# nalcala/MIDASPOM

Hardware: AMD Instinct MI355X
Metric: grid-point x timestep likelihood evals/sec (higher is better)
Workload: dtype f64; 1 GPU; config2: 64 patches x 50 years, 512x512 (e,c) grid; patches=64, years=50, nvar=8, nstates=256, nextid=40, parallelism=e-row slabs x1, layout=[c][e] (MDP_LAYOUT_CE, the drop-ins' layout)

## Files before the change

midaspom_amd/csrc/spom_engine.h:

```cpp
#ifndef MDP_SPOM_ENGINE_H
#define MDP_SPOM_ENGINE_H

#include <hip/hip_runtime_api.h>
#include <hip/hip_vector_types.h>

#include <cstddef>
#include <cstdint>
#include <map>
#include <mutex>
#include <set>
#include <string>
#include <vector>

#include "mdp_internal.h"
#include "spom_jit.h"

constexpr int kBlock = 256;
constexpr int kEPL = 2;
constexpr int kMaxDeg = 24;
constexpr uint32_t kSubPart = 16;
constexpr uint32_t kOffBits = 22;
constexpr uint32_t kOffMask = (1u << kOffBits) - 1u;
constexpr size_t kFwdLds = 48 * 1024;
constexpr int kZTermsDev = 8;
// ... 17 lines not shown
constexpr int kJitKblockTall = 512;

struct LaunchNote {
    const char *fmt;
    uint64_t a[4];
};

struct DevCtx {
    int device = 0;
    mutable std::vector<LaunchNote> noted;
    hipStream_t stream = nullptr;
    double *S = nullptr;
    uint32_t *var_cols = nullptr, *row_col = nullptr;
    uint32_t *pairA = nullptr, *pairB = nullptr, *pairOff = nullptr;
    uint32_t *udesc = nullptr, *prog = nullptr, *pairPart0 = nullptr, *partP = nullptr, *partK0 = nullptr;
    double *e = nullptr, *c = nullptr;
    size_t cap_e = 0, cap_c = 0;
    uint32_t ne = 0, nc = 0;
    uint32_t ne_sform = 0;
    uint32_t *plist = nullptr;
    size_t cap_plist = 0;
    double *elist = nullptr;
    size_t cap_elist = 0;
    uint32_t nlist = 0, nlist_epl = 0;
    bool plist_identity = true;
    double *ZPV = nullptr, *R = nullptr, *out = nullptr, *gpart = nullptr;
    size_t cap_zpv = 0, cap_r = 0, cap_out = 0, cap_gpart = 0;
    unsigned long long *stamps[3] = {nullptr, nullptr, nullptr};
    size_t cap_st[3] = {0, 0, 0};
    size_t nst[3] = {0, 0, 0};
    double *zs = nullptr, *sv = nullptr, *Qrow = nullptr, *Zg = nullptr;
    double *zsq = nullptr;
    double *zc = nullptr;
    size_t cap_zc = 0;
    uint2 *items = nullptr;
    uint2 *qslot = nullptr;
    uint32_t *qlane = nullptr;
    uint32_t *islot = nullptr;
    uint32_t *itemB = nullptr, *qstart = nullptr, *qitem = nullptr;
    size_t cap_zs = 0, cap_zsq = 0, cap_qrow = 0, cap_zg = 0;
    uint32_t zs_len = 0;
    double *coltab = nullptr;
    size_t cap_coltab = 0;
    uint32_t ct_len = 0;
    uint32_t zs_kmax = 0;
    uint32_t qrows_cb = 1;
// ... 152 lines not shown
inline size_t mmt_lds(const mdp_engine *eng)
{
    const MmtShape sh = mmt_shape(eng);
    return ((sh.db ? 2 : 1) * (size_t)sh.rows * mmt_pts(sh.rt) + 2 * ((size_t)eng->maxA + 1) * mmt_ps(sh.rt)) *
           sizeof(double);
}

inline size_t hs_lds(const mdp_engine *eng)
{
    return (((size_t)1 << eng->hs_nb) + eng->hs_nb + 1) * mmt_pts(eng->hs_rt) * sizeof(double);
}

inline size_t qrows_lds(const mdp_engine *eng, uint32_t cb)
{
    const size_t nv = eng->nvar <= 8 ? 8 : eng->nvar <= 16 ? 16 : 24;
    return ((((size_t)cb * eng->nj + 1) & ~(size_t)1) + (size_t)eng->nj * (cb * nv + 2) + (size_t)cb * eng->npl_slots) *
               sizeof(double) +
           ((size_t)eng->ncoef_d + 1 + eng->qitem.size()) * sizeof(uint32_t);
}

inline size_t fused_lds(const mdp_engine *eng, size_t ct_len)
{
    const size_t fc = (size_t)eng->jit_plan.fused_cols;
    return (ct_len + 2 + fc * (eng->nj + eng->nitems + 2 * eng->ldQ)) * sizeof(double);
}

inline size_t wide_lds(const mdp_engine *eng) { return 2 * ((size_t)eng->maxA + 1) * kBlock * sizeof(double); }


int parse_engine_opts(const char *s, EngineOpts &o, bool diag_build);

enum class MdpPlanMode {
    Compile,
    OfflineCheck,
    TablesOnly
};
int mdp_plan_engine(mdp_engine *eng, const mdp_problem *p, size_t lds_max, MdpPlanMode mode, double *jit_t);

void z_split(const mdp_engine *eng, uint32_t js, double cmax, std::vector<double> &large, double *coef,
             std::vector<uint32_t> *cols = nullptr);
std::string jit_source(mdp_engine *eng, int variant);
int jit_build(mdp_engine *eng, int variant);
int jit_build_chunks(mdp_engine *eng);

#endif
```

midaspom_amd/csrc/spom_engine.hip:

```cpp
#include <hip/hip_ext.h>
#include <hip/hip_runtime.h>

#include <algorithm>
#include <chrono>
#include <cmath>
#include <cstdarg>
#include <cstdio>
#include <cstdlib>
#include <cstring>
#include <mutex>
#include <new>
#include <string>
#include <vector>

#include "spom_dev.h"
#include "spom_engine.h"

namespace {

constexpr int kZpvJ = 64;
constexpr int kZpvSlices = 4;
constexpr int kZpvCT = 2;
constexpr int kZpvUnroll = 8;
constexpr int kStampSlots = 8;
// ... 943 lines not shown
        uint32_t g = 0;
        for (uint32_t i = i0; i < i1; i += kQGroup, ++g) {
            double sg = pl[qitem[i]];
            for (uint32_t u = 1; u < kQGroup && i + u < i1; ++u) sg = sg + pl[qitem[i + u]];
#pragma unroll
            for (int l = 0; l < kQLevels; ++l) {
                if ((g >> l) & 1u) {
                    sg = lev[l] + sg;
                } else {
                    lev[l] = sg;
                    break;
                }
            }
        }
        bool have = false;
#pragma unroll
        for (int l = 0; l < kQLevels; ++l)
            if ((g >> l) & 1u) {
                a = have ? lev[l] + a : lev[l];
                have = true;
            }
    }
    Q[(size_t)(c0 + cl) * ldQ + q] = a;
}

typedef double mdp_d4 __attribute__((ext_vector_type(4)));
template <int NPM>
__global__ __launch_bounds__(kMmaThreads) void k_fwd_mma(
    const double *__restrict__ Q, uint32_t ldQ, const uint32_t *__restrict__ np, const uint2 *__restrict__ kt,
    const uint32_t *__restrict__ kbase, const uint32_t *__restrict__ desc, const uint32_t *__restrict__ dbase,
    const uint2 *__restrict__ wplan, uint32_t tmax, double prior0, const double *__restrict__ evals, uint32_t ne,
    uint32_t c0, uint32_t maxA, uint32_t ktmax, uint32_t zslot, double *__restrict__ out, uint32_t ld_out,
    uint32_t out_cs)
{
    constexpr uint32_t PTS = mma_pts(NPM), ROWS = mma_rows(NPM), PS = mma_ps(NPM), RT = PTS / 16;
    static_assert(NPM <= (int)ROWS && NPM <= 256, "state rows");
    extern __shared__ __attribute__((aligned(16))) double mlds[];
    double *Va = mlds, *Vb = mlds + (size_t)ROWS * PTS;
    double *xp = Vb + (size_t)ROWS * PTS, *yp = xp + (size_t)(maxA + 1) * PS;
    const uint32_t lane = threadIdx.x & 63u, wv = __builtin_amdgcn_readfirstlane(threadIdx.x >> 6);
    const uint32_t p0 = blockIdx.x * PTS, ic = c0 + blockIdx.y;
    if (threadIdx.x < PTS) {
        const uint32_t ie = p0 + threadIdx.x;
        const double e = ie < ne ? evals[ie] : 0.0;
        const double x = e > 1.0 ? 1.0 : e, y = 1.0 - x;
        double a = 1.0, b = 1.0;
// ... 1033 lines not shown

int qrows_attrs(const mdp_engine *eng, DevCtx &d)
{
    if (d.qrows_attr_set) return MDP_OK;
    const size_t lds_max = qrows_lds(eng, kQrowsMaxC);
    if (lds_max > 64 * 1024)
        for (const void *fn : {(const void *)k_qrows<8, true, 1>, (const void *)k_qrows<8, false, 1>,
                               (const void *)k_qrows<16, false, 1>, (const void *)k_qrows<24, false, 1>,
                               (const void *)k_qrows<8, true, 2>, (const void *)k_qrows<8, false, 2>,
                               (const void *)k_qrows<16, false, 2>, (const void *)k_qrows<8, true, 4>,
                               (const void *)k_qrows<8, false, 4>})
            HIP_TRY(hipFuncSetAttribute(fn, hipFuncAttributeMaxDynamicSharedMemorySize,
                                        (int)std::min(lds_max, kQrowsLdsMax)));
    d.qrows_attr_set = true;
    return MDP_OK;
}

void free_device(DevCtx &d)
{
    (void)hipSetDevice(d.device);
    void *ptrs[] = {d.S, d.var_cols, d.row_col, d.pairA, d.pairB, d.pairOff, d.udesc, d.prog,
                    d.pairPart0, d.partP, d.partK0, d.e, d.c, d.ZPV, d.R, d.out, d.gpart,
                    d.zs, d.zsq, d.sv, d.Qrow, d.Zg, d.coltab, d.items, d.itemB, d.qstart, d.qitem,
                    d.Pg, d.V, d.np_d, d.udesc_w, d.zc, d.plist, d.elist, d.qslot, d.qlane, d.islot,
                    d.mma_kt, d.mma_kbase, d.mma_desc, d.mma_dbase, d.mma_wplan,
                    d.mmt_kt, d.mmt_ktile, d.mmt_wplan, d.mmt_cidx,
                    d.hs_kt, d.hs_cidx, d.hs_pbase, d.hs_ppos, d.hs_dpos, d.hs_dbase, d.hs_pk,
                    d.hs_wplan, d.hs_pass, d.hs_dpk,
                    d.stamps[0], d.stamps[1], d.stamps[2]};
    for (void *ptr : ptrs)
        if (ptr) (void)hipFree(ptr);
    for (hipEvent_t ev : d.ev) (void)hipEventDestroy(ev);
    for (hipModule_t m : d.jit_mod)
        if (m) (void)hipModuleUnload(m);
    for (hipModule_t m : d.cmod) (void)hipModuleUnload(m);
    for (uint32_t *q : d.cqidx)
        if (q) (void)hipFree(q);
    if (d.vscr) (void)hipFree(d.vscr);
    if (d.stream) (void)hipStreamDestroy(d.stream);
}

std::vector<uint32_t> point_list(const double *e, uint32_t ne, uint32_t epl)
{
    std::vector<uint32_t> s_rows, t_rows;
    for (uint32_t i = 0; i < ne; ++i) {
        const double x = e[i] > 1.0 ? 1.0 : e[i], y = 1.0 - x;
        (x >= y ? t_rows : s_rows).push_back(i);
// ... 102 lines not shown
        uint32_t cb = nc >= 1024 ? 4u : nc >= 512 ? 2u : 1u;
        cb = std::min(cb, eng->nvar <= 8 ? 4u : eng->nvar <= 16 ? 2u : 1u);
        while (cb > 1 && qrows_lds(eng, cb) > kQrowsLdsMax) cb >>= 1;
        d.qrows_cb = cb;
    } else if ((rc = dev_grow(d.ZPV, d.cap_zpv, (size_t)nc * (eng->nvar + 1) * eng->nstates)) ||
               (rc = dev_grow(d.R, d.cap_r, (size_t)nc * ldR_of(eng)))) {
        return rc;
    }
    if (!eng->jit && !eng->wide && !eng->lds_part &&
        (rc = dev_grow(d.gpart, d.cap_gpart, (size_t)nc * eng->partP.size() * (eng->nvar + 1))))
        return rc;
    if (eng->diag) {
        d.nst[0] = eng->jit ? (size_t)nc
                            : (size_t)((eng->nstates + kZpvJ - 1) / kZpvJ) * ((nc + kZpvCT - 1) / kZpvCT);
        d.nst[1] = nc;
        d.nst[2] = (size_t)nc * ((ne + kBlock - 1) / kBlock);
        for (int k = 0; k < 3; ++k) {
            if ((rc = dev_grow(d.stamps[k], d.cap_st[k], d.nst[k] * kStampSlots))) return rc;
            HIP_TRY(hipMemset(d.stamps[k], 0, d.cap_st[k] * sizeof(unsigned long long)));
        }
    }
    if (ne) HIP_TRY(hipMemcpy(d.e, e, ne * sizeof(double), hipMemcpyHostToDevice));
    if (nc) HIP_TRY(hipMemcpy(d.c, c, nc * sizeof(double), hipMemcpyHostToDevice));
    d.ne = ne;
    d.nc = nc;
    return MDP_OK;
}

template <int NP, int DEG, int EPL>
void launch_fwd_epl(const mdp_engine *eng, const DevCtx &d, double *out, OutStrides os, hipStream_t s)
{
    uint32_t se = os.se, sc = os.sc;
    dim3 grid(d.nc, (d.ne + kBlock * EPL - 1) / (kBlock * EPL));
    const uint32_t nprog = (uint32_t)eng->prog.size() - 1;
    note_launch(eng, d, "%s<%d,%d,%d>", eng->fwd_lds ? "k_forward_lds" : "k_forward", NP, DEG, EPL);
    if (eng->fwd_lds)
        MDP_LAUNCH((k_forward_lds<NP, DEG, EPL>), grid, dim3(kBlock), eng->fwd_lds_bytes, s,
                           d.R, ldR_of(eng), d.prog, nprog, eng->np[0], eng->prior0, d.e, d.ne, out, se,
                           sc, d.stamps[2]);
    else
        MDP_LAUNCH((k_forward<NP, DEG, EPL>), grid, dim3(kBlock), 0, s, d.R, ldR_of(eng),
                           d.prog, nprog, eng->np[0], eng->prior0, d.e, d.ne, out, se, sc);
}

template <int NP, int DEG>
void launch_fwd(const mdp_engine *eng, const DevCtx &d, double *out, OutStrides os, hipStream_t s)
// ... 30 lines not shown
        const double *cv = d.c, *ctab = d.coltab;
        uint32_t ctl = d.ct_len, kmax = d.zs_kmax;
        double *vscr = d.vscr;
        uint32_t ldv = d.ldv;
        const uint32_t *qidx = nullptr;
        uint32_t se = os.se, sc = os.sc;
        const uint32_t kb = d.fused ? eng->jit_kblock_fused : d.tall ? (uint32_t)kJitKblockTall : eng->jit_kblock;
        const uint32_t pro = d.fused ? eng->jit_pro_fused : 1u;
        const uint32_t epl = d.fused ? (uint32_t)eng->jit_epl_fused : (uint32_t)eng->jit_epl;
        const uint32_t spl = eng->jit_plan.vlds && (eng->jit_plan.vsplit == 2 || eng->jit_plan.vsplit == 4)
                                 ? (uint32_t)eng->jit_plan.vsplit : 1u;
        const uint32_t *plist = epl > 1 && !d.plist_identity ? d.plist : nullptr;
        uint32_t nlist = epl > 1 ? d.nlist : d.ne;
        if (epl > 1 && ((!plist && !d.plist_identity) || d.nlist_epl % epl))
            return mdp_set_error(MDP_EINVAL, "no point list for %u points per lane", epl);
        const uint64_t gy = (nlist + kb * epl - 1) / (kb * epl);
        const uint32_t fc = d.fused ? (uint32_t)eng->jit_plan.fused_cols : 1u;
        const uint64_t nb = gy * ((d.nc + fc - 1) / fc);
        if (nb * kb * fc * spl > 0xffffffffull)
            return mdp_set_error(MDP_EUNSUPPORTED, "grid %u x %u too large", d.ne, d.nc);
        const double *tab = d.fused ? ctab : Qrow;
        if (plist) ev = d.elist;
        uint32_t nblk = (uint32_t)nb;
        void *args[] = {(void *)&tab,   (void *)&cv,   (void *)&ev,  (void *)&ctl,  (void *)&nlist,
                        (void *)&ne,    (void *)&nc,   (void *)&plist, (void *)&nblk, (void *)&kmax,
                        (void *)&one,   (void *)&qidx, (void *)&out, (void *)&se,   (void *)&sc,
                        (void *)&prior0, (void *)&vscr, (void *)&ldv, (void *)&st};
        if (!eng->chunks.empty()) {
            const size_t nch = d.cfn.size();
            if (nch != eng->chunks.size() || d.cqidx.size() != nch)
                return mdp_set_error(MDP_EHIP, "forward chunks not loaded (%zu of %zu)", nch, eng->chunks.size());
            for (size_t i = 0; i < nch; ++i) {
                qidx = d.cqidx[i];
                HIP_TRY(hipExtModuleLaunchKernel(d.cfn[i], (uint32_t)(nb * kb * spl), 1, 1, kb * spl, 1, 1, 0, s, args,
                                                 nullptr, i == 0 ? t_kev.start : nullptr,
                                                 i + 1 == nch ? t_kev.stop : nullptr, 0));
            }
            note_launch(eng, d, "mdp_fwd_jit<reading,maxA%u,chunks%zu%s>", eng->maxA, nch,
                        eng->chunks[0].qidx.empty() ? "" : ",gather");
            return MDP_OK;
        }
        const uint32_t dyn = d.fused ? (d.ct_len + 2) * (uint32_t)sizeof(double) : 0u;
        HIP_TRY(hipExtModuleLaunchKernel(d.jit_fn[d.fused ? 1 : d.tall ? 2 : 0], (uint32_t)(nb * kb * fc * spl * pro), 1, 1,
                                         kb * fc * spl * pro, 1, 1, dyn, s, args, nullptr, t_kev.start, t_kev.stop, 0));
        note_launch(eng, d, "mdp_fwd_jit<%s,maxA%u>", d.fused ? "fused" : "reading", eng->maxA);
        if (d.tall) note_launch(eng, d, "mdp_fwd_jit<reading,kb%d>", kJitKblockTall);
// ... 634 lines not shown
```

midaspom_amd/csrc/spom_jit.cpp:

```cpp
#include <dlfcn.h>
#include <hip/hip_runtime_api.h>
#include <hip/hiprtc.h>
#include <unistd.h>

#include <cstdio>
#include <cstdlib>
#include <cstring>
#include <map>
#include <set>
#include <atomic>
#include <mutex>
#include <sstream>
#include <algorithm>
#include <cstdint>
#include <string>
#include <sys/stat.h>
#include <type_traits>
#include <vector>

#include "spom_jit.h"

extern "C" hipError_t hipRuntimeGetVersion(int *) __attribute__((weak));

namespace {
// ... 323 lines not shown
         "    double *__restrict__ out, u32 ld_out, u32 out_cs, double prior0,\n"
         "    double *__restrict__ vscr, u32 ldv, unsigned long long *__restrict__ stamps)\n{\n"
      << "    __shared__ __attribute__((aligned(16))) double Ql[2 * FC * LDQ + 2];\n"
      << stamp(6) << stamp(0);
    if (pl.fused) {
        o << "    extern __shared__ __attribute__((aligned(16))) double ct[];\n"
             "    const u32 n2 = ct_len / 2;\n";
        for (uint32_t k = 0; k < nstg; ++k)
            o << "    const u32 si" << k << "_ = threadIdx.x + " << k << " * NT;\n"
              << "    const double2 stg" << k << "_ = ((const double2 *)coltab)[si" << k << "_ < n2 ? si" << k << "_ : 0];\n";
    }
    o <<
         "    const u32 nb = nblk, full = nb & ~7u;\n"
      << (pl.xcd ? "    const u32 lb = blockIdx.x < full ? (blockIdx.x & 7u) * (full >> 3) + (blockIdx.x >> 3) : blockIdx.x;\n"
                 : "    const u32 lb = blockIdx.x + 0 * full;\n") <<
         "    const u32 half = threadIdx.x / KBLOCK, tid = threadIdx.x % KBLOCK;\n"
      << (FC > 1 && SPL == 1 && pl.rot ? "    const u32 tip = (tid + half * (KBLOCK / 2)) % KBLOCK;\n" : "    const u32 tip = tid;\n")
      << (pl.efast ? "    const u32 gy = (nlist + KBLOCK * EPL - 1) / (KBLOCK * EPL), ic0 = lb / gy * FC, by = lb % gy;\n"
                   : "    const u32 ncb = (nc + FC - 1) / FC, ic0 = lb % ncb * FC, by = lb / ncb;\n")
      << (SPL > 1 || FC == 1 ? "    const u32 ic = ic0;\n" : "    const u32 ic = ic0 + half;\n")
      << (SPL > 1 ? "    const double *Qh = Ql;\n" : "    const double *Qh = Ql + half * LDQ;\n");
    const std::string front = std::string(
         "    u32 ie[EPL], pp[EPL];\n    bool st[EPL];\n    double ev[EPL];\n") +
         (EPL == 1 ? "    pp[0] = by * KBLOCK + tip;\n"
                     "    ie[0] = pp[0];\n"
                     "    st[0] = ie[0] < ne;\n"
                     "    ev[0] = evals[st[0] ? ie[0] : 0u];\n"
                   : "    u32 q_[EPL];\n"
                     "#pragma unroll\n"
                     "    for (int i = 0; i < EPL; ++i) {\n"
                     "        pp[i] = by * (KBLOCK * EPL) + tip * EPL + i;\n"
                     "        q_[i] = pp[i] < nlist ? pp[i] : 0x80000000u;\n"
                     "        const u32 j_ = q_[i] & 0x7fffffffu;\n"
                     "        ev[i] = evals[plist ? (pp[i] < nlist ? pp[i] : nlist) : (j_ < ne ? j_ : 0u)];\n"
                     "    }\n"
                     "    if (plist) {\n"
                     "#pragma unroll\n"
                     "        for (int i = 0; i < EPL; ++i) {\n"
                     "            const u32 l_ = plist[pp[i] < nlist ? pp[i] : 0u];\n"
                     "            q_[i] = pp[i] < nlist ? l_ : 0x80000000u;\n"
                     "        }\n"
                     "    }\n"
                     "#pragma unroll\n"
                     "    for (int i = 0; i < EPL; ++i) {\n"
                     "        ie[i] = q_[i] & 0x7fffffffu;\n"
                     "        st[i] = !(q_[i] >> 31) && ie[i] < ne;\n"
                     "    }\n") +
         "#pragma unroll\n"
         "    for (int i = 0; i < EPL; ++i) ev[i] = ie[i] < ne ? ev[i] : 0.0;\n"
         "    asm volatile(\"\" :: \"s\"(kmax), \"s\"(one), \"s\"(out), \"s\"(ld_out), \"s\"(out_cs), \"s\"(prior0), "
         "\"s\"(vscr), \"s\"(ldv));\n";
    std::string wblock;
    {
        std::ostringstream w;
        w << "#pragma unroll\n"
             "    for (int i = 0; i < EPL; ++i) {\n"
             "        const double e = ev[i];\n"
             "        xx[i] = e > 1.0 ? 1.0 : e;\n"
             "        yy[i] = 1.0 - xx[i];\n"
             "    }\n"
             "    const bool tf = xx[0] >= yy[0];\n"
             "    const double *Qp = Qh + (tf ? FC * LDQ : 0);\n"
             "#pragma unroll\n"
             "    for (int i = 0; i < EPL; ++i) {\n"
             "        const double num = tf ? yy[i] : xx[i], den = tf ? xx[i] : yy[i];\n"
             "        zz[i] = num / den;\n"
             "        bb[i] = den;\n"
             "        const double g = tf ? 1.0 : zz[i];\n"
             "        bp[i][0] = 1.0;\n"
             "        gp[i][0] = 1.0;\n"
             "#pragma unroll\n        for (int r = 1; r <= DP; ++r) bp[i][r] = bp[i][r - 1] * den;\n"
             "#pragma unroll\n        for (int r = 1; r <= DG; ++r) gp[i][r] = gp[i][r - 1] * g;\n";
        const char *vdst = pl.vlds ? "Vl[(k * EPL + i) * KBLOCK + tid]" : "v[i][k]";
        const char *kloop = SPL > 1 ? "#pragma unroll\n        for (int k = half; k < NPMAX; k += SPL) "
                                    : "#pragma unroll\n        for (int k = 0; k < NPMAX; ++k) ";
        if (pl.first)
            w << kloop << vdst << " = k < " << np0 << " ? 1.0 : 0.0;\n";
        else
            w << kloop << vdst << " = k < " << np0 << " ? vscr[((size_t)k * nc + ic) * ldv + pp[i]] : 0.0;\n";
        w << "    }\n";
        wblock = w.str();
    }
    const bool w_early = !pl.fused && !pl.first;
    const std::string early_w = w_early ? wblock : std::string();
    o << "    double xx[EPL], yy[EPL], zz[EPL], bb[EPL], bp[EPL][DP + 1], gp[EPL][DG + 1];\n"
         "    double v[EPL][NPMAX];\n    double n[EPL][(NPMAX + SPL - 1) / SPL];\n";
    if (pl.vlds)
        o << "    __shared__ double Vl[NPMAX * EPL * KBLOCK];\n";
    auto vref = [&](uint32_t k) {
        return pl.vlds ? "Vl[(" + std::to_string(k) + " * EPL + i) * KBLOCK + tid]" : "v[i][" + std::to_string(k) + "]";
    };
    if (!pl.fused && !gather) {
        const uint32_t nk = (uint32_t)((ldq_local / 2 + nt_all - 1) / nt_all);
        o << "    const double2 *src_ = (const double2 *)(Qrow + (size_t)ic * LDQ);\n"
             "    constexpr u32 N2 = LDQ / 2;\n";
        for (uint32_t k = 0; k < nk; ++k) {
            const std::string K = std::to_string(k);
            o << "    const u32 qi" << K << "_ = threadIdx.x + " << K << " * NT;\n"
              << "    const double2 qt" << K << "_ = src_[qi" << K << "_ < N2 ? qi" << K << "_ : 0];\n"
              << "    const u32 ra" << K << "_ = REVQ[qi" << K << "_ < N2 ? 2 * qi" << K << "_ : 0], rb" << K
              << "_ = REVQ[qi" << K << "_ < N2 ? 2 * qi" << K << "_ + 1 : 0];\n";
        }
        o << front << early_w << "    {\n        double2 *dst_ = (double2 *)Ql;\n";
        for (uint32_t k = 0; k < nk; ++k) {
            const std::string K = std::to_string(k);
            o << "        dst_[qi" << K << "_ < N2 ? qi" << K << "_ : LDQ] = qt" << K << "_;\n"
              << "        Ql[qi" << K << "_ < N2 ? LDQ + ra" << K << "_ : 2 * LDQ] = qt" << K << "_.x;\n"
// ... 6 lines not shown
        for (uint32_t k = 0; k < nk; ++k) {
            const std::string K = std::to_string(k);
            o << "    const u32 qi" << K << "_ = threadIdx.x + " << K << " * NT;\n"
              << "    const u32 qx" << K << "_ = qidx[qi" << K << "_ < NQG ? qi" << K << "_ : 0];\n"
              << "    const u32 qr" << K << "_ = REVQ[qi" << K << "_ < NQG ? qi" << K << "_ : 0];\n";
        }
        o << front;
        for (uint32_t k = 0; k < nk; ++k) o << "    const double qt" << k << "_ = src_[qx" << k << "_];\n";
        o << early_w;
        for (uint32_t k = 0; k < nk; ++k) {
            const std::string K = std::to_string(k);
            o << "    Ql[qi" << K << "_ < NQG ? qi" << K << "_ : 2 * LDQ] = qt" << K << "_;\n"
              << "    Ql[qi" << K << "_ < NQG ? LDQ + qr" << K << "_ : 2 * LDQ] = qt" << K << "_;\n";
        }
        o << stamp(1);
    } else {
        o << "    double cc[FC];\n"
             "#pragma unroll\n"
             "    for (int f = 0; f < FC; ++f) cc[f] = cvals[ic0 + f < nc ? ic0 + f : 0u];\n"
          << front <<
             "#pragma unroll\n"
             "    for (int f = 0; f < FC; ++f) cc[f] = ic0 + f < nc ? cc[f] : 0.0;\n"
          <<
             "    __shared__ double Zl[FC * NJ];\n"
             "#define PLS (NITEMS + 1)\n"
             "    __shared__ double Pl[FC * PLS];\n"
          <<
             "    const uint2 *Itl = (const uint2 *)(ct + OFF_IT);\n"
             "    const u32 *Qsl = (const u32 *)(ct + OFF_QS);\n"
             "    const u32 *Qil = (const u32 *)(ct + OFF_QI);\n"
             "    const u32 *Rql = (const u32 *)(ct + OFF_RQ);\n"
             "    const double *zcl = ct + OFF_ZC;\n"
             "    const double *Svl = ct;\n"
             "    const double *zl = ct + OFF_ZS;\n";
        for (uint32_t k = 0; k < nstg; ++k)
            o << "    ((double2 *)ct)[si" << k << "_ < n2 ? si" << k << "_ : n2] = stg" << k << "_;\n";
        o << "    __syncthreads();\n"
          << stamp(4);
        o <<
             "    constexpr int KPC = (FC * NITEMS + NT - 1) / NT;\n"
             "    constexpr int KQ = (FC * LDQ + NT - 1) / NT;\n"
             "    double Fp[KPC];\n"
             "    u32 zi[KPC];\n"
             "#define ITEM_W(k) ((k) * NT + (((k) & 1) ? threadIdx.x : NT - 1 - threadIdx.x))\n"
             "#define ZW(k) ((k) * NT + threadIdx.x)\n#define QW(k) ((k) * NT + threadIdx.x)\n"
"#pragma unroll\n"
             "    for (int k = 0; k < KPC; ++k) {\n"
             "        const u32 w = ITEM_W(k);\n"
             "        Fp[k] = 0.0;\n"
             "        zi[k] = 0u;\n"
             "        if (w >= FC * NITEMS) continue;\n"
             "        const u32 col = w % FC, it = w / FC;\n"
             "        const double c = cc[col];\n"
             "        const uint2 t = Itl[it];\n"
             "        const u32 r = (t.x >> 24) | ((t.y >> 24) << 8), B = t.x & 0xffffffu, j = t.y & 0xffffffu;\n"
             "        double f[NVAR];\n"
             "        const u32 nB = ~B;\n"
             "        (void)j;\n"
             "#pragma unroll\n"
             "        for (int b = 0; b < NVAR; ++b) {\n"
             "            const u32 bit = NVAR - 1 - b;\n"
             "            const double p = fmin(c * Svl[r * NVAR + b], 1.0);\n"
             "            f[b] = (double)((nB >> bit) & 1u) - p;\n"
             "        }\n"
             "#pragma unroll\n"
             "        for (int b = 0; b < NVAR; b += 2) f[b] = b + 1 < NVAR ? fabs(f[b]) * fabs(f[b + 1]) : fabs(f[b]);\n"
             "#pragma unroll\n"
             "        for (int s = 2; s < NVAR; s *= 2)\n"
             "#pragma unroll\n"
             "            for (int b = 0; b + s < NVAR; b += 2 * s) f[b] *= f[b + s];\n"
             "        Fp[k] = f[0];\n"
             "        zi[k] = col * NJ + r;\n"
             "    }\n"
             "    u32 qb[KQ], qn[KQ], qx[KQ][QUN];\n"
             "#pragma unroll\n"
             "    for (int k = 0; k < KQ; ++k) {\n"
             "        const u32 w = QW(k), q = w % LDQ;\n"
             "        const bool live = w < FC * LDQ && q < NCOEF;\n"
             "        const u32 q0 = live ? Qsl[q] : 0u, q1 = live ? Qsl[q + 1] : 0u;\n"
             "        qb[k] = q0;\n"
             "        qn[k] = q1 - q0;\n"
             "#pragma unroll\n"
             "        for (int u = 0; u < QUN; ++u) { const u32 t_ = Qil[q0 + u]; qx[k][u] = (u32)u < qn[k] ? t_ : (u32)NITEMS; }\n"
             "    }\n"
             "#pragma unroll\n"
             "    for (int k = 0; k < (FC * NJ + NT - 1) / NT; ++k) {\n"
             "        const u32 w = ZW(k);\n"
             "        if (w < FC * NJ) {\n"
             "            const u32 col = w % FC, r = w / FC;\n"
             "            const double c = cc[col];\n"
             "            double sk[KZ];\n"
             "#pragma unroll\n"
             "            for (u32 kk = 0; kk < KZ; kk += 2) {\n"
             "                const double2 t2 = ((const double2 *)zl)[(ZPAD || kk < kmax ? kk : kk % 8u) / 2 * NJ + r];\n"
             "                sk[kk] = t2.x;\n"
             "                sk[kk + 1] = t2.y;\n"
             "            }\n"
             "            double za = 1.0, zb = 1.0, zc = 1.0, zd = 1.0;\n"
             "#pragma unroll\n"
             "            for (u32 kk = 0; kk < KZ; kk += 8) {\n"
             "                const bool in = ZPAD || kk < kmax;\n"
             "#pragma unroll\n"
             "                for (int u = 0; u < 8; ++u) sk[kk + u] = in ? sk[kk + u] : 0.0;\n"
             "                za *= fma(-c, sk[kk + 0], 1.0) * fma(-c, sk[kk + 4], 1.0);\n"
             "                zb *= fma(-c, sk[kk + 1], 1.0) * fma(-c, sk[kk + 5], 1.0);\n"
             "                zc *= fma(-c, sk[kk + 2], 1.0) * fma(-c, sk[kk + 6], 1.0);\n"
             "                zd *= fma(-c, sk[kk + 3], 1.0) * fma(-c, sk[kk + 7], 1.0);\n"
             "            }\n"
             "            double z = (za * zb) * (zc * zd);\n"
             "            if (kmax && !(fma(-c, sk[0], 1.0) > 0.0)) z = 0.0;\n"
             "            {\n"
             "                const double2 *zq = (const double2 *)(zcl + r * 8);\n"
             "                const double2 p01 = zq[0], p23 = zq[1], p45 = zq[2], p67 = zq[3];\n"
             "                double q = p67.y;\n"
             "                q = fma(q, c, p67.x);\n"
             "                q = fma(q, c, p45.y);\n"
             "                q = fma(q, c, p45.x);\n"
             "                q = fma(q, c, p23.y);\n"
             "                q = fma(q, c, p23.x);\n"
             "                q = fma(q, c, p01.y);\n"
             "                q = fma(q, c, p01.x);\n"
             "                z *= exp(-(q * c));\n"
             "            }\n"
             "            Zl[col * NJ + r] = z;\n"
             "        }\n"
             "    }\n"
             "    __syncthreads();\n"
          << stamp(5) <<
             "#pragma unroll\n"
             "    for (int k = 0; k < KPC; ++k) {\n"
             "        const u32 w = ITEM_W(k);\n"
             "        if (w < FC * NITEMS) Pl[(w % FC) * PLS + w / FC] = Zl[zi[k]] * Fp[k];\n"
             "    }\n"
             "    if (threadIdx.x < FC) Pl[threadIdx.x * PLS + NITEMS] = 0.0;\n"
             "    __syncthreads();\n"
          << stamp(1) <<
             "#pragma unroll\n"
             "    for (int k = 0; k < KQ; ++k) {\n"
             "        const u32 w = QW(k);\n"
             "        if (w < FC * LDQ) {\n"
             "            const double *pl = Pl + (w / LDQ) * PLS;\n"
          << qsum_flat_code(std::max<uint32_t>(1u, pl.qmaxlen), std::min<uint32_t>(std::max<uint32_t>(1u, pl.qmaxlen), 16u)) <<
             "            Ql[w] = a;\n"
             "            Ql[FC * LDQ + (w / LDQ) * LDQ + Rql[w % LDQ]] = a;\n"
             "        }\n"
             "    }\n";
    }
    if (!w_early) o << wblock;
    o << "    __syncthreads();\n"
      << stamp(2)
      << (PRO > 1 ? "    if (threadIdx.x >= NTF) return;\n" : "");
    const bool split_forms = !pl.vlds && pl.split_forms;
    const char *qbase = "Qp";
    bool gmul = true;
    auto hexpr = [&](uint32_t d) {
        const uint32_t off = d & ((1u << 22) - 1u), nX = (d >> 22) & 31u;
        std::string e = std::string(qbase) + "[" + std::to_string(off) + "]";
        for (uint32_t m = 1; m <= nX; ++m)
            e = "fma(" + e + ", zz[i], " + qbase + "[" + std::to_string(off + m) + "])";
        return e;
    };
    auto gfac = [&](uint32_t d) {
        const uint32_t nX = (d >> 22) & 31u, nA = d >> 27;
        return gmul && nA > nX ? " * gp[i][" + std::to_string(nA - nX) + "]" : std::string();
    };
    const int window = pl.window > 0 ? pl.window : 8;
    const char *guard = pl.vlds
        ? "    { u32 g_; asm volatile(\"s_mov_b32 %0, %1\" : \"=s\"(g_) : \"s\"(one) : \"memory\"); if (g_) {\n"
        : "    { u32 g_; asm volatile(\"s_mov_b32 %0, %1\" : \"=s\"(g_) : \"s\"(one)); if (g_) {\n";
    const int nslot = pl.slots > 0 ? pl.slots : 0;
    if (nslot > 0) o << "    double pc[EPL][" << nslot << "];\n";
// ... 423 lines not shown
```

midaspom_amd/csrc/spom_jit.h:

```cpp
#ifndef SPOM_JIT_H
#define SPOM_JIT_H
#include <cstddef>
#include <cstdint>
#include <string>
#include <vector>

struct MdpJitPlan {
    std::vector<uint32_t> np;
    std::vector<uint32_t> udesc;
    size_t ldQ = 0;
    bool fused = false;
    int fused_cols = 2;
    int pro = 1;
    bool fast_log = true;
    bool split_forms = true;
    bool rot = true;
    int hack = 0;
    uint32_t nj = 0, nvar = 0, nitems = 0, ncoef = 0, nqi = 0;
    uint32_t off_it = 0, off_qs = 0, off_qi = 0, off_rq = 0, off_zc = 0, off_zs = 0;
    uint32_t kzmax = 0;
    bool zpad = false;
    uint32_t qmaxlen = 0;
    uint32_t ct_max = 0;
    int epl = 0;
    int kblock = 256;
    bool vlds = false;
    int vsplit = 4;
    int window = 8;
    bool diag = false;
    bool xcd = true;
    bool efast = true;
    int slots = 8;
    int wpe = 0;
    double flops_pt = 0;
    bool first = true, last = true;
    uint32_t e0 = 0;
    std::vector<uint32_t> qidx;
// ... 24 lines not shown
```

midaspom_amd/csrc/spom_plan.cpp:

```cpp
#include <algorithm>
#include <chrono>
#include <cmath>
#include <cstdio>
#include <cstdlib>
#include <cstring>
#include <map>
#include <new>
#include <set>
#include <string>
#include <thread>
#include <unordered_map>
#include <vector>

#include "spom_engine.h"
#include "spom_opts.h"

namespace {
const char *const kEngineOptNames[] = {
    "MDP_JIT", "MDP_FUSED", "MDP_FUSED_COLS", "MDP_EPL", "MDP_JIT_SLOTS", "MDP_JIT_WINDOW", "MDP_JIT_XCD",
    "MDP_JIT_EFAST", "MDP_QROWS_XCD", "MDP_FWD", "MDP_WIDE", "MDP_VSPLIT", "MDP_VLDS_EPL", "MDP_VLDS_MAXUSES",
    "MDP_JIT_CHUNK", "MDP_JIT_GATHER", "MDP_QGLOBAL", "MDP_FAST_LOG", "MDP_JIT_KBLOCK", "MDP_WIDE_CB",
    "MDP_JIT_CHECK", "MDP_JIT_DUMP", "MDP_JIT_THREADS", "MDP_JIT_VERBOSE", "MDP_JIT_SPLIT", "MDP_JIT_ROT",
    "MDP_WIDE_MMA", "MDP_HS_RADIX", "MDP_HS_WAVES"};
const char *const kDiagOptNames[] = {"MDP_DIAG", "MDP_JIT_HACK", "MDP_JIT_WPE", "MDP_HS_PROBE"};
}

int parse_engine_opts(const char *s, EngineOpts &o, bool diag_build)
{
    o.kv.clear();
    if (!s) return MDP_OK;
    return mdp_for_each_opt(s, [&](const std::string &k, const std::string &val, bool has) -> int {
        bool known = false, diag = false;
        for (const char *n : kEngineOptNames) known |= k == n;
        for (const char *n : kDiagOptNames) diag |= k == n;
        if (diag && !diag_build)
            return mdp_set_error(MDP_EINVAL, "option %s is measurement-only (libmidaspom_diag.so, -DMDP_DIAG_BUILD)",
                                 k.c_str());
        if (!known && !diag) return mdp_set_error(MDP_EINVAL, "unknown engine option '%s'", k.c_str());
        o.kv[k] = has ? val : std::string("1");
        return MDP_OK;
    });
}

namespace {

constexpr size_t kLdsBudget = 120 * 1024;
// ... 1064 lines not shown
                plan.kblock = (int)vkb / plan.epl;
                plan.window = 16;
                eng->fused_mode = 0;
                if (const char *sv = eng->opts.get("MDP_VSPLIT")) plan.vsplit = atoi(sv) == 1 ? 1 : atoi(sv) == 2 ? 2 : 4;
            }
            plan.np = eng->np;
            plan.udesc = eng->udesc_d;
            plan.ldQ = eng->ldQ;
            plan.diag = eng->diag;
            if (const char *cv = eng->opts.get("MDP_JIT_SLOTS")) plan.slots = atoi(cv);
            if (const char *wv = eng->opts.get("MDP_JIT_WPE")) plan.wpe = atoi(wv);
            if (const char *xv = eng->opts.get("MDP_JIT_XCD")) plan.xcd = atoi(xv) != 0;
            if (const char *fv2 = eng->opts.get("MDP_JIT_EFAST")) plan.efast = atoi(fv2) != 0;
            if (const char *qx = eng->opts.get("MDP_QROWS_XCD")) eng->qrows_xcd = atoi(qx) != 0;
            if (const char *ev = eng->opts.get("MDP_EPL")) {
                plan.epl = atoi(ev);
                eng->jit_shape_env = true;
            }
            if (const char *wv = eng->opts.get("MDP_JIT_WINDOW")) plan.window = atoi(wv);
            if (const char *fv = eng->opts.get("MDP_FUSED")) eng->fused_mode = atoi(fv) != 0;
            if (const char *cv = eng->opts.get("MDP_FUSED_COLS")) plan.fused_cols = std::max(1, std::min(4, atoi(cv)));
            if (const char *cv = eng->opts.get("MDP_JIT_HACK")) plan.hack = atoi(cv);
            if (const char *cv = eng->opts.get("MDP_FAST_LOG")) plan.fast_log = atoi(cv) != 0;
            if (const char *cv = eng->opts.get("MDP_JIT_KBLOCK"); cv && !vlds) {
                plan.kblock = atoi(cv) == 512 ? 512 : 256;
                eng->jit_shape_env = true;
            }
            plan.nj = eng->nj;
            plan.nvar = eng->nvar;
            plan.nitems = eng->nitems;
            plan.ncoef = eng->ncoef_d;
            plan.nqi = (uint32_t)eng->qitem.size();
            {
                size_t kz = 0;
                std::vector<double> large;
                for (uint32_t js = 0; js < eng->nj; ++js) {
                    z_split(eng, js, 1.0, large, nullptr);
                    kz = std::max(kz, large.size());
                }
                plan.kzmax = (uint32_t)std::max<size_t>(8, (kz + 7) & ~(size_t)7);
            }
            plan.qmaxlen = 0;
            for (size_t q = 0; q + 1 < eng->qstart.size(); ++q)
                plan.qmaxlen = std::max(plan.qmaxlen, eng->qstart[q + 1] - eng->qstart[q]);
            auto even = [](size_t v) { return (uint32_t)((v + 1) & ~(size_t)1); };
            if (const char *sv = eng->opts.get("MDP_JIT_SPLIT")) plan.split_forms = atoi(sv) != 0;
// ... 161 lines not shown
```

Measured before the change: 1723 billion grid-point-timestep evals/s.

## Precompute per-point ratio table and split fused Z exp into separate pass

Adds a device point table built once when the grid is set, holding each e value and its precomputed ratio num/den. The JIT kernel loads both as a double2 instead of doing a per-block division. In fused mode the point set-up moves ahead of the first barrier. A second option splits the fused Z computation into a product pass and a separate exp pass, each with its own LDS row and staggered thread mapping, so the transcendental work is spread across waves and the Q descriptor loads overlap. This costs extra LDS, an extra load per point, and a one-time table kernel with a synchronize.

```diff
diff --git a/midaspom_amd/csrc/spom_engine.h b/midaspom_amd/csrc/spom_engine.h
--- a/midaspom_amd/csrc/spom_engine.h
+++ b/midaspom_amd/csrc/spom_engine.h
@@ -63,6 +63,8 @@
     size_t cap_plist = 0;
     double *elist = nullptr;
     size_t cap_elist = 0;
+    double2 *ptab = nullptr;
+    size_t cap_ptab = 0;
     uint32_t nlist = 0, nlist_epl = 0;
     bool plist_identity = true;
     double *ZPV = nullptr, *R = nullptr, *out = nullptr, *gpart = nullptr;
@@ -261,7 +263,8 @@
 inline size_t fused_lds(const mdp_engine *eng, size_t ct_len)
 {
     const size_t fc = (size_t)eng->jit_plan.fused_cols;
-    return (ct_len + 2 + fc * (eng->nj + eng->nitems + 2 * eng->ldQ)) * sizeof(double);
+    const size_t zrows = eng->jit_plan.zsplit ? 2 : 1;
+    return (ct_len + 2 + fc * (zrows * eng->nj + eng->nitems + 2 * eng->ldQ)) * sizeof(double);
 }
 
 inline size_t wide_lds(const mdp_engine *eng) { return 2 * ((size_t)eng->maxA + 1) * kBlock * sizeof(double); }
diff --git a/midaspom_amd/csrc/spom_engine.hip b/midaspom_amd/csrc/spom_engine.hip
--- a/midaspom_amd/csrc/spom_engine.hip
+++ b/midaspom_amd/csrc/spom_engine.hip
@@ -989,6 +989,19 @@
             }
     }
     Q[(size_t)(c0 + cl) * ldQ + q] = a;
+}
+
+__global__ __launch_bounds__(kBlock) void k_point_table(const double *__restrict__ e, uint32_t n,
+                                                        double2 *__restrict__ tab)
+{
+    const uint32_t i = blockIdx.x * kBlock + threadIdx.x;
+    if (i > n) return;
+    const double ev = i < n ? e[i] : 0.0;
+    const double xx = ev > 1.0 ? 1.0 : ev;
+    const double yy = 1.0 - xx;
+    const bool tf = xx >= yy;
+    const double num = tf ? yy : xx, den = tf ? xx : yy;
+    tab[i] = make_double2(ev, num / den);
 }
 
 typedef double mdp_d4 __attribute__((ext_vector_type(4)));
@@ -2068,7 +2081,7 @@
     void *ptrs[] = {d.S, d.var_cols, d.row_col, d.pairA, d.pairB, d.pairOff, d.udesc, d.prog,
                     d.pairPart0, d.partP, d.partK0, d.e, d.c, d.ZPV, d.R, d.out, d.gpart,
                     d.zs, d.zsq, d.sv, d.Qrow, d.Zg, d.coltab, d.items, d.itemB, d.qstart, d.qitem,
-                    d.Pg, d.V, d.np_d, d.udesc_w, d.zc, d.plist, d.elist, d.qslot, d.qlane, d.islot,
+                    d.Pg, d.V, d.np_d, d.udesc_w, d.zc, d.plist, d.elist, d.ptab, d.qslot, d.qlane, d.islot,
                     d.mma_kt, d.mma_kbase, d.mma_desc, d.mma_dbase, d.mma_wplan,
                     d.mmt_kt, d.mmt_ktile, d.mmt_wplan, d.mmt_cidx,
                     d.hs_kt, d.hs_cidx, d.hs_pbase, d.hs_ppos, d.hs_dpos, d.hs_dbase, d.hs_pk,
@@ -2217,6 +2230,17 @@
     }
     if (ne) HIP_TRY(hipMemcpy(d.e, e, ne * sizeof(double), hipMemcpyHostToDevice));
     if (nc) HIP_TRY(hipMemcpy(d.c, c, nc * sizeof(double), hipMemcpyHostToDevice));
+    if (eng->jit && eng->jit_plan.ptab) {
+        const bool listed = !d.plist_identity;
+        const size_t nl = listed ? (size_t)d.nlist + 1 : 0;
+        if ((rc = dev_grow(d.ptab, d.cap_ptab, (size_t)ne + 1 + nl))) return rc;
+        hipLaunchKernelGGL(k_point_table, dim3(ne / kBlock + 1), dim3(kBlock), 0, d.stream, d.e, ne, d.ptab);
+        if (listed)
+            hipLaunchKernelGGL(k_point_table, dim3(d.nlist / kBlock + 1), dim3(kBlock), 0, d.stream, d.elist, d.nlist,
+                               d.ptab + ne + 1);
+        HIP_TRY(hipGetLastError());
+        HIP_TRY(hipStreamSynchronize(d.stream));
+    }
     d.ne = ne;
     d.nc = nc;
     return MDP_OK;
@@ -2293,6 +2317,7 @@
         const double *tab = d.fused ? ctab : Qrow;
         if (plist) ev = d.elist;
         uint32_t nblk = (uint32_t)nb;
+        if (eng->jit_plan.ptab) ev = (const double *)(plist ? d.ptab + d.ne + 1 : d.ptab);
         void *args[] = {(void *)&tab,   (void *)&cv,   (void *)&ev,  (void *)&ctl,  (void *)&nlist,
                         (void *)&ne,    (void *)&nc,   (void *)&plist, (void *)&nblk, (void *)&kmax,
                         (void *)&one,   (void *)&qidx, (void *)&out, (void *)&se,   (void *)&sc,
diff --git a/midaspom_amd/csrc/spom_jit.cpp b/midaspom_amd/csrc/spom_jit.cpp
--- a/midaspom_amd/csrc/spom_jit.cpp
+++ b/midaspom_amd/csrc/spom_jit.cpp
@@ -369,17 +369,29 @@
       << (SPL > 1 ? "    const double *Qh = Ql;\n" : "    const double *Qh = Ql + half * LDQ;\n");
     const std::string front = std::string(
          "    u32 ie[EPL], pp[EPL];\n    bool st[EPL];\n    double ev[EPL];\n") +
-         (EPL == 1 ? "    pp[0] = by * KBLOCK + tip;\n"
+         (pl.ptab ? "    double zt[EPL];\n" : "") +
+         (EPL == 1 ? std::string(
+                     "    pp[0] = by * KBLOCK + tip;\n"
                      "    ie[0] = pp[0];\n"
-                     "    st[0] = ie[0] < ne;\n"
-                     "    ev[0] = evals[st[0] ? ie[0] : 0u];\n"
-                   : "    u32 q_[EPL];\n"
+                     "    st[0] = ie[0] < ne;\n") +
+                     (pl.ptab ? "    {\n"
+                                "        const double2 ez_ = ((const double2 *)evals)[st[0] ? ie[0] : ne];\n"
+                                "        ev[0] = ez_.x;\n"
+                                "        zt[0] = ez_.y;\n"
+                                "    }\n"
+                              : "    ev[0] = evals[st[0] ? ie[0] : 0u];\n")
+                   : std::string(
+                     "    u32 q_[EPL];\n"
                      "#pragma unroll\n"
                      "    for (int i = 0; i < EPL; ++i) {\n"
                      "        pp[i] = by * (KBLOCK * EPL) + tip * EPL + i;\n"
                      "        q_[i] = pp[i] < nlist ? pp[i] : 0x80000000u;\n"
-                     "        const u32 j_ = q_[i] & 0x7fffffffu;\n"
-                     "        ev[i] = evals[plist ? (pp[i] < nlist ? pp[i] : nlist) : (j_ < ne ? j_ : 0u)];\n"
+                     "        const u32 j_ = q_[i] & 0x7fffffffu;\n") +
+                     (pl.ptab ? "        const double2 ez_ = ((const double2 *)evals)[plist ? (pp[i] < nlist ? pp[i] : nlist)\n"
+                                "                                                          : (pp[i] < nlist && j_ < ne ? j_ : ne)];\n"
+                                "        ev[i] = ez_.x;\n"
+                                "        zt[i] = ez_.y;\n"
+                              : "        ev[i] = evals[plist ? (pp[i] < nlist ? pp[i] : nlist) : (j_ < ne ? j_ : 0u)];\n") +
                      "    }\n"
                      "    if (plist) {\n"
                      "#pragma unroll\n"
@@ -393,14 +405,16 @@
                      "        ie[i] = q_[i] & 0x7fffffffu;\n"
                      "        st[i] = !(q_[i] >> 31) && ie[i] < ne;\n"
                      "    }\n") +
-         "#pragma unroll\n"
-         "    for (int i = 0; i < EPL; ++i) ev[i] = ie[i] < ne ? ev[i] : 0.0;\n"
+         "#pragma unroll\n" +
+         (pl.ptab ? "    for (int i = 0; i < EPL; ++i) ev[i] = pp[i] < nlist && ie[i] < ne ? ev[i] : 0.0;\n"
+                  : "    for (int i = 0; i < EPL; ++i) ev[i] = ie[i] < ne ? ev[i] : 0.0;\n") +
          "    asm volatile(\"\" :: \"s\"(kmax), \"s\"(one), \"s\"(out), \"s\"(ld_out), \"s\"(out_cs), \"s\"(prior0), "
          "\"s\"(vscr), \"s\"(ldv));\n";
     std::string wblock;
     {
         std::ostringstream w;
-        w << "#pragma unroll\n"
+        w << "    // point set-up\n"
+             "#pragma unroll\n"
              "    for (int i = 0; i < EPL; ++i) {\n"
              "        const double e = ev[i];\n"
              "        xx[i] = e > 1.0 ? 1.0 : e;\n"
@@ -410,8 +424,10 @@
              "    const double *Qp = Qh + (tf ? FC * LDQ : 0);\n"
              "#pragma unroll\n"
              "    for (int i = 0; i < EPL; ++i) {\n"
-             "        const double num = tf ? yy[i] : xx[i], den = tf ? xx[i] : yy[i];\n"
-             "        zz[i] = num / den;\n"
+          << (pl.ptab ? "        const double den = tf ? xx[i] : yy[i];\n"
+                        "        zz[i] = zt[i];\n"
+                      : "        const double num = tf ? yy[i] : xx[i], den = tf ? xx[i] : yy[i];\n"
+                        "        zz[i] = num / den;\n") <<
              "        bb[i] = den;\n"
              "        const double g = tf ? 1.0 : zz[i];\n"
              "        bp[i][0] = 1.0;\n"
@@ -425,11 +441,12 @@
             w << kloop << vdst << " = k < " << np0 << " ? 1.0 : 0.0;\n";
         else
             w << kloop << vdst << " = k < " << np0 << " ? vscr[((size_t)k * nc + ic) * ldv + pp[i]] : 0.0;\n";
-        w << "    }\n";
+        w << "    }\n    // end of point set-up\n";
         wblock = w.str();
     }
     const bool w_early = !pl.fused && !pl.first;
     const std::string early_w = w_early ? wblock : std::string();
+    const bool w_stage = pl.fused && pl.ptab;
     o << "    double xx[EPL], yy[EPL], zz[EPL], bb[EPL], bp[EPL][DP + 1], gp[EPL][DG + 1];\n"
          "    double v[EPL][NPMAX];\n    double n[EPL][(NPMAX + SPL - 1) / SPL];\n";
     if (pl.vlds)
@@ -482,7 +499,7 @@
              "#pragma unroll\n"
              "    for (int f = 0; f < FC; ++f) cc[f] = ic0 + f < nc ? cc[f] : 0.0;\n"
           <<
-             "    __shared__ double Zl[FC * NJ];\n"
+             "    __shared__ double Zl[" << (pl.zsplit ? "2 * " : "") << "FC * NJ];\n"
              "#define PLS (NITEMS + 1)\n"
              "    __shared__ double Pl[FC * PLS];\n"
           <<
@@ -495,6 +512,7 @@
              "    const double *zl = ct + OFF_ZS;\n";
         for (uint32_t k = 0; k < nstg; ++k)
             o << "    ((double2 *)ct)[si" << k << "_ < n2 ? si" << k << "_ : n2] = stg" << k << "_;\n";
+        if (w_stage) o << wblock;
         o << "    __syncthreads();\n"
           << stamp(4);
         o <<
@@ -503,7 +521,11 @@
              "    double Fp[KPC];\n"
              "    u32 zi[KPC];\n"
              "#define ITEM_W(k) ((k) * NT + (((k) & 1) ? threadIdx.x : NT - 1 - threadIdx.x))\n"
-             "#define ZW(k) ((k) * NT + threadIdx.x)\n#define QW(k) ((k) * NT + threadIdx.x)\n"
+             "#define ZW(k) ((k) * NT + threadIdx.x)\n"
+          << (pl.zsplit ? "#define ZE0 ((((FC * NJ < NT ? FC * NJ : NT) + 63) / 64 * 64) % NT)\n"
+                          "#define ZEW(k) ((k) * NT + (threadIdx.x + NT - ZE0) % NT)\n"
+                          "#define QW(k) ((k) * NT + (threadIdx.x + NT - (2 * ZE0) % NT) % NT)\n"
+                        : "#define QW(k) ((k) * NT + threadIdx.x)\n") <<
 "#pragma unroll\n"
              "    for (int k = 0; k < KPC; ++k) {\n"
              "        const u32 w = ITEM_W(k);\n"
@@ -531,45 +553,26 @@
              "            for (int b = 0; b + s < NVAR; b += 2 * s) f[b] *= f[b + s];\n"
              "        Fp[k] = f[0];\n"
              "        zi[k] = col * NJ + r;\n"
-             "    }\n"
+             "    }\n";
+        const std::string qdesc = std::string(
              "    u32 qb[KQ], qn[KQ], qx[KQ][QUN];\n"
              "#pragma unroll\n"
              "    for (int k = 0; k < KQ; ++k) {\n"
              "        const u32 w = QW(k), q = w % LDQ;\n"
-             "        const bool live = w < FC * LDQ && q < NCOEF;\n"
+             "        const bool live = w < FC * LDQ && q < NCOEF;\n") +
+             (pl.zsplit ? "        qb[k] = 0u;\n"
+                          "        qn[k] = 0u;\n"
+                          "#pragma unroll\n"
+                          "        for (int u = 0; u < QUN; ++u) qx[k][u] = (u32)NITEMS;\n"
+                          "        if (w >= FC * LDQ) continue;\n"
+                        : "") +
              "        const u32 q0 = live ? Qsl[q] : 0u, q1 = live ? Qsl[q + 1] : 0u;\n"
              "        qb[k] = q0;\n"
              "        qn[k] = q1 - q0;\n"
              "#pragma unroll\n"
              "        for (int u = 0; u < QUN; ++u) { const u32 t_ = Qil[q0 + u]; qx[k][u] = (u32)u < qn[k] ? t_ : (u32)NITEMS; }\n"
-             "    }\n"
-             "#pragma unroll\n"
-             "    for (int k = 0; k < (FC * NJ + NT - 1) / NT; ++k) {\n"
-             "        const u32 w = ZW(k);\n"
-             "        if (w < FC * NJ) {\n"
-             "            const u32 col = w % FC, r = w / FC;\n"
-             "            const double c = cc[col];\n"
-             "            double sk[KZ];\n"
-             "#pragma unroll\n"
-             "            for (u32 kk = 0; kk < KZ; kk += 2) {\n"
-             "                const double2 t2 = ((const double2 *)zl)[(ZPAD || kk < kmax ? kk : kk % 8u) / 2 * NJ + r];\n"
-             "                sk[kk] = t2.x;\n"
-             "                sk[kk + 1] = t2.y;\n"
-             "            }\n"
-             "            double za = 1.0, zb = 1.0, zc = 1.0, zd = 1.0;\n"
-             "#pragma unroll\n"
-             "            for (u32 kk = 0; kk < KZ; kk += 8) {\n"
-             "                const bool in = ZPAD || kk < kmax;\n"
-             "#pragma unroll\n"
-             "                for (int u = 0; u < 8; ++u) sk[kk + u] = in ? sk[kk + u] : 0.0;\n"
-             "                za *= fma(-c, sk[kk + 0], 1.0) * fma(-c, sk[kk + 4], 1.0);\n"
-             "                zb *= fma(-c, sk[kk + 1], 1.0) * fma(-c, sk[kk + 5], 1.0);\n"
-             "                zc *= fma(-c, sk[kk + 2], 1.0) * fma(-c, sk[kk + 6], 1.0);\n"
-             "                zd *= fma(-c, sk[kk + 3], 1.0) * fma(-c, sk[kk + 7], 1.0);\n"
-             "            }\n"
-             "            double z = (za * zb) * (zc * zd);\n"
-             "            if (kmax && !(fma(-c, sk[0], 1.0) > 0.0)) z = 0.0;\n"
-             "            {\n"
+             "    }\n";
+        const char *zexp =
              "                const double2 *zq = (const double2 *)(zcl + r * 8);\n"
              "                const double2 p01 = zq[0], p23 = zq[1], p45 = zq[2], p67 = zq[3];\n"
              "                double q = p67.y;\n"
@@ -580,17 +583,65 @@
              "                q = fma(q, c, p23.x);\n"
              "                q = fma(q, c, p01.y);\n"
              "                q = fma(q, c, p01.x);\n"
-             "                z *= exp(-(q * c));\n"
+             "                const double ez = exp(-(q * c));\n";
+        if (!pl.zsplit) o << qdesc;
+        o <<
+             "#pragma unroll\n"
+             "    for (int k = 0; k < (FC * NJ + NT - 1) / NT; ++k) {\n"
+             "        const u32 w = ZW(k);\n"
+             "        if (w < FC * NJ) {\n"
+             "            const u32 col = w % FC, r = w / FC;\n"
+             "            const double c = cc[col];\n"
+             "            double sk[KZ];\n"
+             "#pragma unroll\n"
+             "            for (u32 kk = 0; kk < KZ; kk += 2) {\n"
+             "                const double2 t2 = ((const double2 *)zl)[(ZPAD || kk < kmax ? kk : kk % 8u) / 2 * NJ + r];\n"
+             "                sk[kk] = t2.x;\n"
+             "                sk[kk + 1] = t2.y;\n"
              "            }\n"
-             "            Zl[col * NJ + r] = z;\n"
-             "        }\n"
-             "    }\n"
+             "            double za = 1.0, zb = 1.0, zc = 1.0, zd = 1.0;\n"
+             "#pragma unroll\n"
+             "            for (u32 kk = 0; kk < KZ; kk += 8) {\n"
+             "                const bool in = ZPAD || kk < kmax;\n"
+             "#pragma unroll\n"
+             "                for (int u = 0; u < 8; ++u) sk[kk + u] = in ? sk[kk + u] : 0.0;\n"
+             "                za *= fma(-c, sk[kk + 0], 1.0) * fma(-c, sk[kk + 4], 1.0);\n"
+             "                zb *= fma(-c, sk[kk + 1], 1.0) * fma(-c, sk[kk + 5], 1.0);\n"
+             "                zc *= fma(-c, sk[kk + 2], 1.0) * fma(-c, sk[kk + 6], 1.0);\n"
+             "                zd *= fma(-c, sk[kk + 3], 1.0) * fma(-c, sk[kk + 7], 1.0);\n"
+             "            }\n"
+             "            double z = (za * zb) * (zc * zd);\n"
+             "            if (kmax && !(fma(-c, sk[0], 1.0) > 0.0)) z = 0.0;\n";
+        if (!pl.zsplit)
+            o << "            {\n" << zexp <<
+                 "                z *= ez;\n"
+                 "            }\n"
+                 "            Zl[col * NJ + r] = z;\n"
+                 "        }\n"
+                 "    }\n";
+        else
+            o << "            Zl[col * NJ + r] = z;\n"
+                 "        }\n"
+                 "    }\n"
+                 "#pragma unroll\n"
+                 "    for (int k = 0; k < (FC * NJ + NT - 1) / NT; ++k) {\n"
+                 "        const u32 w = ZEW(k);\n"
+                 "        if (w < FC * NJ) {\n"
+                 "            const u32 col = w % FC, r = w / FC;\n"
+                 "            const double c = cc[col];\n"
+                 "            {\n" << zexp <<
+                 "                Zl[FC * NJ + col * NJ + r] = ez;\n"
+                 "            }\n"
+                 "        }\n"
+                 "    }\n" << qdesc;
+        o <<
              "    __syncthreads();\n"
           << stamp(5) <<
              "#pragma unroll\n"
              "    for (int k = 0; k < KPC; ++k) {\n"
              "        const u32 w = ITEM_W(k);\n"
-             "        if (w < FC * NITEMS) Pl[(w % FC) * PLS + w / FC] = Zl[zi[k]] * Fp[k];\n"
+          << (pl.zsplit ? "        if (w < FC * NITEMS) Pl[(w % FC) * PLS + w / FC] = (Zl[zi[k]] * Zl[FC * NJ + zi[k]]) * Fp[k];\n"
+                        : "        if (w < FC * NITEMS) Pl[(w % FC) * PLS + w / FC] = Zl[zi[k]] * Fp[k];\n") <<
              "    }\n"
              "    if (threadIdx.x < FC) Pl[threadIdx.x * PLS + NITEMS] = 0.0;\n"
              "    __syncthreads();\n"
@@ -606,7 +657,7 @@
              "        }\n"
              "    }\n";
     }
-    if (!w_early) o << wblock;
+    if (!w_early && !w_stage) o << wblock;
     o << "    __syncthreads();\n"
       << stamp(2)
       << (PRO > 1 ? "    if (threadIdx.x >= NTF) return;\n" : "");
diff --git a/midaspom_amd/csrc/spom_jit.h b/midaspom_amd/csrc/spom_jit.h
--- a/midaspom_amd/csrc/spom_jit.h
+++ b/midaspom_amd/csrc/spom_jit.h
@@ -13,6 +13,8 @@
     int fused_cols = 2;
     int pro = 1;
     bool fast_log = true;
+    bool ptab = true;
+    bool zsplit = true;
     bool split_forms = true;
     bool rot = true;
     int hack = 0;
diff --git a/midaspom_amd/csrc/spom_plan.cpp b/midaspom_amd/csrc/spom_plan.cpp
--- a/midaspom_amd/csrc/spom_plan.cpp
+++ b/midaspom_amd/csrc/spom_plan.cpp
@@ -21,7 +21,7 @@
     "MDP_JIT_EFAST", "MDP_QROWS_XCD", "MDP_FWD", "MDP_WIDE", "MDP_VSPLIT", "MDP_VLDS_EPL", "MDP_VLDS_MAXUSES",
     "MDP_JIT_CHUNK", "MDP_JIT_GATHER", "MDP_QGLOBAL", "MDP_FAST_LOG", "MDP_JIT_KBLOCK", "MDP_WIDE_CB",
     "MDP_JIT_CHECK", "MDP_JIT_DUMP", "MDP_JIT_THREADS", "MDP_JIT_VERBOSE", "MDP_JIT_SPLIT", "MDP_JIT_ROT",
-    "MDP_WIDE_MMA", "MDP_HS_RADIX", "MDP_HS_WAVES"};
+    "MDP_WIDE_MMA", "MDP_HS_RADIX", "MDP_HS_WAVES", "MDP_POINT_TABLE", "MDP_FUSED_ZSPLIT"};
 const char *const kDiagOptNames[] = {"MDP_DIAG", "MDP_JIT_HACK", "MDP_JIT_WPE", "MDP_HS_PROBE"};
 }
 
@@ -1132,6 +1132,8 @@
             if (const char *cv = eng->opts.get("MDP_FUSED_COLS")) plan.fused_cols = std::max(1, std::min(4, atoi(cv)));
             if (const char *cv = eng->opts.get("MDP_JIT_HACK")) plan.hack = atoi(cv);
             if (const char *cv = eng->opts.get("MDP_FAST_LOG")) plan.fast_log = atoi(cv) != 0;
+            if (const char *cv = eng->opts.get("MDP_POINT_TABLE")) plan.ptab = atoi(cv) != 0;
+            if (const char *cv = eng->opts.get("MDP_FUSED_ZSPLIT")) plan.zsplit = atoi(cv) != 0;
             if (const char *cv = eng->opts.get("MDP_JIT_KBLOCK"); cv && !vlds) {
                 plan.kblock = atoi(cv) == 512 ? 512 : 256;
                 eng->jit_shape_env = true;
```

Result: no change. 1734 billion grid-point-timestep evals/s (median of 4 runs) (+0.7%).
